# nanoporetech/vbz_compression

Measured on AMD Instinct MI355X. Metric: MB/s encode+decode, int16 signal, 1/2/4/8 MI355X vs CPU; ratio preserved, higher is better.
Workload: dtype int16

## Files before the change

### vbz_compression_amd/csrc/vbz_api.hip

```cpp
#include <hip/hip_runtime.h>

#include <cmath>
#include <cstdarg>
#include <cstdio>
#include <cstdlib>
#include <cstring>
#include <condition_variable>
#include <deque>
#include <mutex>
#include <optional>
#include <string>
#include <map>
#include <vector>

#include "../../include/vbz.h"
#include "../../include/vbz_gpu.h"
#include "vbz_kernels.h"
#include "scratch_tables.h"

using namespace vbzhip;


struct ProfEntry
{
// ... 2122 lines not shown
        return -2;
    }
    Timed t(c, "sized_layout");
    HIPCHK(c, launch_sized_layout(n, (const uint8_t*)bt->src, bt->src_off, bt->src_size, bt->src_bytes, align, raw_size, raw_off, c->stream),
           "sized layout launch");
    return 0;
}

int vbz_gpu_synth_lengths(vbz_gpu_ctx* c, uint64_t seed, uint64_t first, uint32_t n, uint32_t* out_len)
{
    if (!c) return -1;
    DeviceGuard dg(c->device);
    HIPCHK(c, launch_synth_lengths(seed, first, n, out_len, c->stream), "synth_lengths launch");
    return 0;
}

int vbz_gpu_synth_signal(vbz_gpu_ctx* c, uint64_t seed, uint64_t first, uint32_t n, void* dst, const uint64_t* off,
                         const uint32_t* len)
{
    if (!c) return -1;
    DeviceGuard dg(c->device);
    HIPCHK(c, launch_synth_signal(seed, first, n, (uint8_t*)dst, off, len, c->stream), "synth_signal launch");
    return 0;
}

int vbz_gpu_synth_u32(vbz_gpu_ctx* c, uint64_t seed, uint64_t first, uint32_t n, void* dst, const uint64_t* off, const uint32_t* len)
{
    if (!c) return -1;
    DeviceGuard dg(c->device);
    HIPCHK(c, launch_synth_u32(seed, first, n, (uint8_t*)dst, off, len, c->stream), "synth_u32 launch");
    return 0;
}

#ifdef VBZ_EXPERIMENTS
VBZ_EXPORT size_t vbz_gpu_x_plan_bytes(void) { return sizeof(EncPlan); }
VBZ_EXPORT int vbz_gpu_x_svb_handover(vbz_gpu_ctx* c, const vbz_gpu_batch* bt, void* plans_out)
{
    if (!c || !bt || !plans_out) return -1;
    DeviceGuard dg(c->device);
    const uint32_t n = bt->n_reads;
    if (n == 0) return 0;
    hipStream_t s = c->stream;
    ReadBatch rb = to_rb(bt);
    uint32_t num, den;
    svb_factor(2, true, &num, &den);
    const size_t scratch_need = (size_t)(((unsigned __int128)bt->src_bytes * num + den - 1) / den) + (size_t)n * 96 + 256;
    StageSlots m;
    if (!ensure(c, c->scratch, scratch_need) || !ensure_carved(c, c->meta, m, n) || !ensure(c, c->encplan, zstd_encode_plan_bytes(n))) return -1;
    uint64_t* const svb_off = m.svb_off;
    uint32_t *const svb_cap = m.svb_cap, *const svb_size = m.svb_size, *const gate = m.gate;
    HIPCHK(c, launch_plan_scratch(n, bt->src_size, num, den, c->scratch.cap, svb_off, svb_cap, gate, false, s), "plan launch");
    ReadBatch a = rb;
    a.dst = (uint8_t*)c->scratch.p;
    a.dst_off = svb_off;
    a.dst_cap = svb_cap;
    a.result = svb_size;
    a.gate = gate;
    HIPCHK(c, launch_svb_encode(a, 2, true, 0, false, false, nullptr, c->encplan.p, s), "svb_encode launch");
    ReadBatch cp = rb;
    cp.src = (const uint8_t*)c->scratch.p;
    cp.src_off = svb_off;
    cp.src_size = svb_size;
    cp.gate = gate;
    HIPCHK(c, launch_copy_bytes(cp, 0, s), "copy launch");
    HIPCHK(c, hipMemcpyAsync(plans_out, c->encplan.p, (size_t)n * sizeof(EncPlan), hipMemcpyDeviceToDevice, s), "plan copy");
    return 0;
}
VBZ_EXPORT int vbz_gpu_x_runs_counts(vbz_gpu_ctx* c, unsigned long long* out4, int reset)
{
    if (!c || !out4) return -1;
    DeviceGuard dg(c->device);
    HIPCHK(c, hipStreamSynchronize(c->stream), "runs counts sync");
    HIPCHK(c, zstd_fast_runs_counts(out4, reset != 0), "runs counts");
    return 0;
}
VBZ_EXPORT int vbz_gpu_x_streams_counts(vbz_gpu_ctx* c, unsigned long long* out3, int reset)
{
    if (!c || !out3) return -1;
    DeviceGuard dg(c->device);
    HIPCHK(c, hipStreamSynchronize(c->stream), "streams counts sync");
    HIPCHK(c, zstd_fast_streams_counts(out3, reset != 0), "streams counts");
    return 0;
}
#endif

void vbz_gpu_profile_enable(vbz_gpu_ctx* c, int enable)
{
    if (!c) return;
    if (!enable) drain_profile(c);
    c->profiling = enable != 0;
    if (c->half) vbz_gpu_profile_enable(c->half, enable);
}

int vbz_gpu_decode_span_paths(vbz_gpu_ctx* c, uint32_t* by_spans)
{
    if (!c) return -1;
    DeviceGuard guard(c->device);
    if (by_spans) *by_spans = 0;
    if (c->last_span_frames == 0) return 0;
    std::vector<uint32_t> redo(c->last_span_frames);
    if (hipMemcpyAsync(redo.data(), c->last_span_redo, 4ull * redo.size(), hipMemcpyDeviceToHost, c->stream) != hipSuccess) return -1;
    if (hipStreamSynchronize(c->stream) != hipSuccess) return -1;
    uint32_t nb = 0;
    for (uint32_t v : redo) nb += v == 0;
    if (by_spans) *by_spans = nb;
    return (int)c->last_span_frames;
}

static int decode_paths_one(vbz_gpu_ctx* c, uint32_t* batched, uint32_t* walked);

int vbz_gpu_decode_paths(vbz_gpu_ctx* c, uint32_t* batched, uint32_t* walked)
{
    if (!c) return -1;
    uint32_t b0 = 0, w0 = 0, b1 = 0, w1 = 0;
    const int n0 = decode_paths_one(c, &b0, &w0);
    const int n1 = (n0 >= 0 && c->last_split && c->half) ? decode_paths_one(c->half, &b1, &w1) : 0;
    if (batched) *batched = b0 + b1;
    if (walked) *walked = w0 + w1;
    return (n0 < 0 || n1 < 0) ? -1 : n0 + n1;
}

int vbz_gpu_decode_literals_ahead(vbz_gpu_ctx* c)
{
    if (!c) return -1;
    int total = 0;
    for (vbz_gpu_ctx* k : { c, (c->last_split && c->half) ? c->half : (vbz_gpu_ctx*)nullptr }) {
        if (!k || !k->last_frames || !k->last_walked || !zstd_ref_literals_enabled() || !k->reflits.p) continue;
        DeviceGuard guard(k->device);
        const uint32_t per = k->last_lit_units;
        if (per == 0) continue;
        std::vector<RefLits> lits((size_t)k->last_frames * per);
        if (hipMemcpyAsync(lits.data(), zstd_ref_lits(k->reflits.p, k->last_frames), sizeof(RefLits) * lits.size(), hipMemcpyDeviceToHost, k->stream) != hipSuccess ||
            hipStreamSynchronize(k->stream) != hipSuccess) {
            (void)hipGetLastError();
            return -1;
        }
        if (k->knobs.trace) {
            std::vector<uint32_t> sk((size_t)k->last_frames * per);
            if (hipMemcpy(sk.data(), zstd_ref_lit_skip(k->reflits.p, k->last_frames), 4 * sk.size(), hipMemcpyDeviceToHost) == hipSuccess)
                for (uint32_t u = 0; u < per; ++u) {
                    uint32_t made = 0, done = 0;
                    for (uint32_t i = 0; i < k->last_frames; ++i) {
                        made += sk[(size_t)u * k->last_frames + i] == 0;
                        done += lits[(size_t)u * k->last_frames + i].blk != 0;
                    }
                    fprintf(stderr, "vbz_hip: literals beside the walk, unit %u: %u made by the scan, %u done\n", u, made, done);
                }
        }
        for (uint32_t i = 0; i < k->last_frames; ++i) {
            bool any = false;
            for (uint32_t u = 0; u < per; ++u) any = any || lits[(size_t)u * k->last_frames + i].blk != 0;
            total += any;
        }
    }
    return total;
}

static int decode_paths_one(vbz_gpu_ctx* c, uint32_t* batched, uint32_t* walked)
{
    DeviceGuard guard(c->device);
    if (batched) *batched = 0;
    if (walked) *walked = 0;
    const uint32_t n = c->last_frames;
    if (n == 0) return 0;
    std::vector<uint32_t> redo(n);
    std::vector<RefPre> pre(c->last_walked ? n : 0);
// ... 357 lines not shown
```

### vbz_compression_amd/csrc/vbz_kernels.h

```cpp
#pragma once

#include <hip/hip_runtime.h>
#include <stdint.h>

namespace vbzhip {

constexpr uint32_t E_ZSTD = 0xFFFFFFFFu;
constexpr uint32_t E_INPUT_SIZE = 0xFFFFFFFEu;
constexpr uint32_t E_INTEGER_SIZE = 0xFFFFFFFDu;
constexpr uint32_t E_DESTINATION_SIZE = 0xFFFFFFFCu;
constexpr uint32_t E_STREAM = 0xFFFFFFFBu;
constexpr uint32_t E_VERSION = 0xFFFFFFFAu;
constexpr uint32_t E_OOM = 0xFFFFFFF9u;
constexpr uint32_t E_DEVICE = 0xFFFFFFF8u;
constexpr uint32_t E_FIRST = E_DEVICE;
constexpr uint32_t GATE_SKIP = E_FIRST - 1u;
constexpr int PHASE_SLOTS = 12;

constexpr uint32_t SIG_NONE = 0, SIG_F32 = 1, SIG_F16 = 2, SIG_BF16 = 3;
constexpr uint32_t SIG_CHUNK = 4;
constexpr uint32_t SIG_COUNT = 8;
constexpr uint32_t SIG_RANGE = 16;
constexpr uint32_t SIG_TRIM = 32;
constexpr uint32_t SIG_WINDOW = 64;
// ... 283 lines not shown
{
    hipStream_t stream = nullptr;
    hipEvent_t fork = nullptr, join = nullptr;
};
typedef SideStream FastSide;
struct SpanEncodeWork
{
    uint64_t stream_bytes = 0;
    void* meta = nullptr;
    uint8_t* tmp = nullptr;
    uint32_t shared_span_bytes = 0;
};
size_t zstd_span_meta_bytes(uint64_t stream_bytes, uint32_t n_reads, uint32_t shared_span_bytes);
uint64_t zstd_span_tmp_bytes(uint64_t stream_bytes, uint32_t n_reads);
uint32_t zstd_span_shared_bytes(uint64_t stream_bytes);
hipError_t launch_zstd_encode_spans(const ReadBatch& b, const ZstdEncodeArgs& a, const SpanEncodeWork& w, hipStream_t s);
hipError_t launch_zstd_encode_matcher(const ReadBatch& b, const ZstdEncodeArgs& a, uint32_t max_raw, const uint32_t* gate_in, uint32_t* gate_out,
                                      hipStream_t s);
hipError_t launch_zstd_decode(const ReadBatch& b, uint32_t toosmall_code, unsigned long long* dbg, const void* seq_dtables,
                              hipStream_t s);
constexpr uint32_t REF_MAXBLK = 4;
struct RefBlock
{
    uint32_t pos;
    uint32_t nseq;
    uint32_t rec_lo, rec_hi;
    uint32_t rep[3];
    uint32_t end;
};
struct RefPre
{
    uint32_t ok, nblk;
    uint32_t why;
    uint32_t tab_cycles, chain_cycles, nseq_last;
    uint32_t pad[2];
    RefBlock blk[REF_MAXBLK];
};
struct RefLits
{
    uint32_t blk, regen, csize, at;
    uint32_t tb, pcap;
    uint32_t tail, pad;
};
struct RefChains
{
    const RefPre* pre = nullptr;
    const void* recs = nullptr;
    const RefLits* lits = nullptr;
    const uint32_t* lits_pos = nullptr;
    uint32_t lits_units = 0;
};

size_t zstd_ref_pre_bytes(uint32_t n_reads);
const RefPre* zstd_ref_pre(const void* pre_meta);
size_t zstd_ref_table_bytes(uint32_t n_reads);
hipError_t launch_zstd_ref_chain(const ReadBatch& b, const uint32_t* redo, void* pre_meta, void* tables, void* recs, uint64_t recs_cap, RefChains* out,
                                 hipStream_t s);
hipError_t launch_zstd_decode_only(const ReadBatch& b, uint32_t toosmall_code, const void* seq_dtables, const uint32_t* only, RefChains chains,
                                   unsigned long long* dbg, hipStream_t s);
size_t zstd_fast_meta_bytes(uint32_t n_reads);
const RefLits* zstd_ref_lits(const void* lit_meta, uint32_t n_reads);
bool zstd_ref_literals_enabled();
const uint32_t* zstd_fast_redo(const void* meta, uint32_t n_reads);
struct RefWork
{
    void *pre = nullptr, *tables = nullptr, *recs = nullptr;
    uint64_t recs_cap = 0;
    void* lits = nullptr;
    uint32_t lit_units = 0;
};
struct FastDecodeArgs
{
    uint32_t toosmall_code = 0;
    const void* seq_dtables = nullptr;
    void* meta = nullptr;
    RefWork ref;
    unsigned long long* dbg = nullptr;
    FastSide side;
};
hipError_t launch_zstd_decode_fast(const ReadBatch& b, const FastDecodeArgs& a, hipStream_t s);
#ifdef VBZ_EXPERIMENTS
hipError_t zstd_fast_runs_counts(unsigned long long out[4], bool reset);
hipError_t zstd_fast_streams_counts(unsigned long long out[3], bool reset);
#endif
size_t zstd_ref_lit_meta_bytes(uint32_t n_reads);
uint32_t zstd_ref_lit_units();
const uint32_t* zstd_ref_lit_skip(const void* lit_meta, uint32_t n_reads);
size_t seq_dtables_bytes();
void seq_dtables_build(void* host_buffer);
struct SpanDecodeArgs
{
    uint32_t toosmall_code = 0;
    const void* seq_dtables = nullptr;
    uint64_t content_bytes = 0;
    void* meta = nullptr;
    const uint32_t* redo = nullptr;
};
size_t zstd_dspan_meta_bytes(uint64_t content_bytes, uint32_t n_reads);
hipError_t launch_zstd_decode_spans(const ReadBatch& b, SpanDecodeArgs* a, hipStream_t s);

hipError_t launch_xxh64_batch(const uint8_t* src, const uint64_t* off, const uint32_t* len, const uint32_t* gate, const uint32_t* skip, uint32_t n,
                              uint64_t* out, hipStream_t s);
hipError_t launch_xxh64_verify(const ReadBatch& b, hipStream_t s);
hipError_t launch_checksum_insert(const ReadBatch& b, const uint64_t* hash, uint32_t hdr, const uint32_t* raw_size, uint32_t integer_size, hipStream_t s);

hipError_t launch_pack_layout(uint32_t n, const uint32_t* result, const uint64_t* dst_off, const uint32_t* dst_cap, uint64_t dst_bytes, uint32_t align,
                              uint64_t* packed_off, uint32_t* packed_size, hipStream_t s);
hipError_t launch_sized_layout(uint32_t n, const uint8_t* src, const uint64_t* src_off, const uint32_t* src_size, uint64_t src_bytes, uint32_t align,
                               uint32_t* raw_size, uint64_t* raw_off, hipStream_t s);
hipError_t launch_pack_gather(uint32_t n, const uint8_t* dst, const uint64_t* dst_off, const uint64_t* packed_off, const uint32_t* packed_size,
                              uint8_t* packed, uint64_t packed_cap, hipStream_t s);

hipError_t launch_plan_scratch(uint32_t n, const uint32_t* raw_size, uint32_t mul_num, uint32_t mul_den, uint64_t limit,
                               uint64_t* off, uint32_t* cap, uint32_t* gate, bool gate_is_input, hipStream_t s);
struct ScratchPlan
{
    uint32_t num, den;
    uint64_t limit;
    uint64_t* off;
    uint32_t* cap;
    uint32_t* gate;
};
hipError_t launch_seg_plan(uint32_t n, const uint32_t* size, uint32_t unit_bytes, const uint32_t* gate, uint32_t max_segs, uint32_t* seg_first,
                           uint32_t* gate_out, const ScratchPlan* scratch, hipStream_t s);
hipError_t launch_count_nonzero(const uint32_t* a, uint32_t n, uint32_t* out, hipStream_t s);
hipError_t launch_canon_classify(uint32_t n, const uint32_t* raw_size, const uint32_t* gate, uint32_t min_bytes, uint32_t* gate_small, uint32_t* gate_large,
                                 uint32_t* counts, hipStream_t s);
struct RoutedTable
{
    uint64_t* src_off = nullptr;
    uint32_t* src_size = nullptr;
    uint64_t* dst_off = nullptr;
    uint32_t *dst_cap = nullptr, *gate = nullptr, *map = nullptr;
    float2* cal = nullptr;
    uint64_t* row = nullptr;
    uint32_t* count = nullptr;
};
struct RouteArgs
{
    const uint32_t* raw_size = nullptr;
    uint32_t min_bytes = 0, max_reads = 0;
    uint64_t max_bytes = 0;
    uint32_t* gate_small = nullptr;
    RoutedTable large;
    uint32_t* cand = nullptr;
};
hipError_t launch_route_reads(const ReadBatch& b, const RouteArgs& a, hipStream_t s);
size_t route_cand_words();
hipError_t launch_route_results(const uint32_t* l_result, const uint32_t* l_map, const uint32_t* l_count, uint32_t max_reads, uint32_t* result, hipStream_t s);
hipError_t launch_parse_sized(uint32_t n, const uint8_t* src, const uint64_t* src_off, const uint32_t* src_size,
                              const uint32_t* dst_cap, const uint32_t* gate_in, uint64_t* pay_off, uint32_t* pay_size, uint32_t* orig_size,
                              uint32_t* gate, hipStream_t s);
hipError_t launch_hand_back(const uint32_t* result, const uint8_t* src, uint32_t* host, uint32_t host_cap, uint32_t seq, uint32_t* ticket, hipStream_t s);
hipError_t launch_validate_batch(uint32_t n, const uint64_t* src_off, const uint32_t* src_size, uint64_t src_bytes, const uint64_t* dst_off,
                                 const uint32_t* dst_cap, uint64_t dst_bytes, uint32_t* gate, hipStream_t s);
hipError_t launch_signal_slots(uint32_t n, const uint64_t* dst_off, const uint32_t* dst_cap, uint32_t elem, const float* offset, const float* scale,
                               uint64_t* off16, uint32_t* cap16, float2* cal, uint32_t* gate, hipStream_t s);
hipError_t launch_chunk_slots(uint32_t n, const uint32_t* cap16, const float* offset, const float* scale, uint32_t L, uint32_t S,
                              const uint64_t* chunk_first, uint64_t chunk_rows, float2* cal, uint32_t* gate, const SignalOut* sig, hipStream_t s);
hipError_t launch_range_samples(uint32_t n, const uint32_t* samples, const uint32_t* begin, const uint32_t* end, uint32_t* range_samples, hipStream_t s);
hipError_t launch_chunk_layout(uint32_t n, const uint32_t* samples, uint32_t L, uint32_t S, uint32_t* count, uint64_t* chunk_first, hipStream_t s);
hipError_t launch_chunk_info(uint32_t n, const uint32_t* samples, uint32_t L, uint32_t S, uint32_t mode, uint32_t end_align, const uint64_t* chunk_first,
                             uint32_t* info, uint64_t info_cap, hipStream_t s);
hipError_t launch_copy_bytes(const ReadBatch& b, uint32_t hdr, hipStream_t s);
hipError_t launch_synth_lengths(uint64_t seed, uint64_t first, uint32_t n, uint32_t* out_len, hipStream_t s);
hipError_t launch_synth_signal(uint64_t seed, uint64_t first, uint32_t n, uint8_t* dst, const uint64_t* off,
// ... 59 lines not shown
```

### vbz_compression_amd/csrc/zstd_encode.hip

```cpp
#include "vbz_kernels.h"
#include "zstd_entropy.h"
#include "zstd_frame.h"

namespace vbzhip {

namespace {

constexpr int WAVE = 64;
constexpr uint32_t BLOCK_MAX = 128u << 10;
constexpr uint32_t MIN_BLOCK = 4096;
constexpr uint32_t HUF_BLOCK_MAX = 92u << 10;
constexpr uint32_t SPLIT_MIN = 2048;
constexpr int MAXBLK = 16;
#ifndef VBZ_SPAN_BLOCK_KB
#define VBZ_SPAN_BLOCK_KB 16
#endif
constexpr uint32_t SPAN_BLOCK = VBZ_SPAN_BLOCK_KB << 10;
#ifndef VBZ_SPAN_SMALL_BLOCKS
#define VBZ_SPAN_SMALL_BLOCKS 2
#endif
constexpr uint32_t SPAN_BYTES_SMALL = SPAN_BLOCK * VBZ_SPAN_SMALL_BLOCKS, SPAN_BYTES_LARGE = SPAN_BLOCK * MAXBLK;
constexpr uint32_t SPAN_LARGE_FROM = 256u << 20;
#ifndef VBZ_KEYSPAN_KB
#define VBZ_KEYSPAN_KB 8
// ... 1959 lines not shown
    }
    const uint32_t cap = b.dst_cap[r];
    uint8_t* out = b.dst + b.dst_off[r];
    if (deep_d) {
        uint32_t hint = deep_d[r];
        if (hint) {
            bool ok = false;
            if (K != 0 && src_cap && seqtab && N - K >= 8192) {
                DeepLayout dl;
                if (hint == RUN_D) hint = run_period(in + K, N - K, lane);
                ok = deep_layout(N, K, in, src_cap[r], out, cap, hdr, dl) && period_holds(in + K, N - K, hint, lane);
            }
            if (lane == 0) deep_d[r] = ok ? hint : 0u;
            if (ok) return;
        }
    }
    if ((uint64_t)hdr + 9 > cap) return;
    const uint32_t S0 = K ? K : N;
    uint32_t nrec = 0, Lit = 0;
    const uint2* rec = nullptr;
    if (src_cap && seqtab && S0 >= 256 && S0 <= BLOCK_MAX) {
        const uint32_t slot = src_cap[r];
        const uint32_t recs_all = S0 / RMIN + 2u + 2u;
        const uint64_t need = (uint64_t)N + 16 + 8ull * recs_all;
        if (need <= slot) {
            uint8_t* ws = const_cast<uint8_t*>(in) + ((slot - 8u * recs_all) & ~7u);
            PT(0);
            tokenise_runs<false>(const_cast<uint8_t*>(in), S0, reinterpret_cast<uint2*>(ws), Lit, nrec, nullptr, lane);
            __syncthreads();
            PT(1);
            rec = reinterpret_cast<const uint2*>(ws);
            if (lane == 0) {
                FP->tok_nrec = nrec;
                FP->tok_lit = Lit;
                FP->tok_done = 1;
            }
        }
    }
    if ((nrec != 0) != guess) return;
    if (nrec) {
        const uint64_t room = 24ull + 8ull * nrec;
        if (room + 4096u > cap) return;
        const uint32_t so = (uint32_t)((cap - room) & ~15ull);
        TokSeqLds& L = LL.ts;
        {
            const uint32_t* g = reinterpret_cast<const uint32_t*>(seqtab);
            uint32_t* l = reinterpret_cast<uint32_t*>(&L.seq);
            for (uint32_t i = lane; i < sizeof(SeqCTables) / 4; i += WAVE) l[i] = g[i];
        }
        wave_lds_sync();
        const uint32_t sb = encode_zero_run_sequences(L, out + so, rec, nrec, lane, 0u);
        wave_lds_sync();
        FP->cp[lane] = L.cp[lane];
        if (lane == 0) {
            FP->seqBytes = sb;
            FP->seqOff = so;
            FP->cpCount = L.cpCount;
            FP->cpSpacing = L.cpSpacing;
        }
        wave_lds_sync();
        PT(2);
    }
    const uint32_t S = nrec ? Lit : S0;
    const uint32_t nblk = nrec ? 1u : (S + T - 1) / T;
    PT(0);
    const bool ok = plan_region_table<TIMED>(LL.tb, FP, 0, in, S, nblk, nrec != 0, nrec, false, lane, tph, tlast);
    __syncthreads();
    if (ok && lane == 0) atomicOr(&pstate[r], PLAN_OPEN | PLAN_REG0 | (K == 0 ? PLAN_REG1 : 0u));
    timed_out();
}
#undef PT

#ifndef VBZ_PACK_TABLE_COPIES
#define VBZ_PACK_TABLE_COPIES 1
#endif
constexpr int PACK_COPIES = VBZ_PACK_TABLE_COPIES;
struct PackLds
{
    uint32_t ctable[PACK_COPIES * 256];
    uint32_t tree[34];
    uint32_t ssize[WAVE], sbeg[WAVE], scnt[WAVE];
    uint32_t obuf[2][OBUF_WORDS];
};

template <bool TIMED>
__device__ __forceinline__ bool pack_region(PackLds& L, const uint8_t* rin, uint32_t r0, uint8_t* out, uint32_t& opos, uint32_t limit, const uint32_t* ctable_g,
                                            const uint32_t* tree_g, uint32_t S, uint32_t nblk, uint32_t treeSize, bool seqmode, bool lastRegion,
                                            uint32_t seqBytes, uint32_t seqOff, int lane, unsigned long long (&tph)[PHASE_SLOTS], unsigned long long& tlast)
{
#define PPHASE(k) do { if (TIMED) { unsigned long long tn = __builtin_readcyclecounter(); tph[k] += tn - tlast; tlast = tn; } } while (0)
#define REDO() return false
    wave_lds_sync();
#pragma unroll
    for (int j = 0; j < 4; ++j) {
        const uint32_t e = ctable_g[lane + 64 * j];
#pragma unroll
        for (int cpy = 0; cpy < PACK_COPIES; ++cpy) L.ctable[256 * cpy + lane + 64 * j] = e;
    }
    const uint32_t* const mytable = L.ctable + 256 * (lane / (WAVE / PACK_COPIES));
    if (lane < 34) L.tree[lane] = tree_g[lane];
    const uint32_t base = S / nblk, extra = S % nblk;
    {
        const uint32_t bj = (uint32_t)(lane >> 2);
        const int q = lane & 3;
        const bool active = bj < nblk;
        uint32_t bs = 0, boff = 0;
        if (active) {
            bs = base + (bj < extra ? 1u : 0u);
            boff = bj * base + (bj < extra ? bj : extra);
        }
        const bool single = bs < 256;
        const uint32_t seg = single ? bs : (bs + 3) >> 2;
        uint32_t cnt = 0;
        if (active) {
            if (single) cnt = q == 0 ? bs : 0;
            else cnt = q < 3 ? seg : bs - 3 * seg;
        }
        L.sbeg[lane] = active ? (cnt ? boff + (uint32_t)q * seg : boff + bs) : S;
        L.scnt[lane] = cnt;
        L.ssize[lane] = 0;
    }
    for (int i = lane; i < 2 * OBUF_WORDS; i += WAVE) (&L.obuf[0][0])[i] = 0;
    wave_lds_sync();
    auto s_cnt = [&](uint32_t i) { return (uint32_t)__builtin_amdgcn_readfirstlane((int)L.scnt[i]); };
    auto s_beg = [&](uint32_t i) { return (uint32_t)__builtin_amdgcn_readfirstlane((int)L.sbeg[i]); };
    const uint32_t nb = (uint32_t)__builtin_amdgcn_readfirstlane((int)nblk);
    uint32_t st = 0;
    while (st < 4 * nb && s_cnt(st) == 0) ++st;
    uint32_t done = 0;
#if VBZ_PACK_PREFETCH
    uint32_t cur[STEP_DW], nxt[STEP_DW];
#else
    uint32_t cur[STEP_DW];
#endif
    auto load_chunk = [&](uint32_t sbeg, uint32_t scount, uint32_t dn, uint32_t (&w)[STEP_DW]) {
#pragma unroll
        for (int k = 0; k < STEP_DW; ++k) w[k] = 0;
        const int32_t room = (int32_t)(scount - dn) - STEP_LANE * lane;
        if (room > 0) {
            const uint8_t* p = rin + sbeg + room - STEP_LANE;
            const bool headroom = (uint64_t)r0 + sbeg >= (uint32_t)STEP_LANE;
            if (room >= STEP_LANE || headroom) {
                uint4 v0;
                __builtin_memcpy(&v0, p, 16);
                w[0] = v0.x; w[1] = v0.y; w[2] = v0.z; w[3] = v0.w;
            } else {
#pragma unroll
                for (int k = 0; k < STEP_LANE; ++k) {
                    const uint32_t byte = (room - STEP_LANE + k >= 0) ? (uint32_t)p[k] : 0u;
                    w[k >> 2] |= byte << (8 * (k & 3));
                }
            }
        }
    };
    auto blk_bs = [&](uint32_t j) { return base + (j < extra ? 1u : 0u); };
    auto blk_lh = [&](uint32_t j) {
        const uint32_t jbs = blk_bs(j);
        const uint32_t worst = (j == 0 ? treeSize : 0u) + 6u + ((jbs * 11u + 7u) >> 3) + 4u;
        const uint32_t big = jbs > worst ? jbs : worst;
        return 3u + (big >= 1024u ? 1u : 0u) + (big >= 16384u ? 1u : 0u);
    };
    auto block_headers = [&](uint32_t j, uint32_t at, uint32_t seqB) {
        if (lane == 0) {
            const uint32_t jbs = blk_bs(j);
            const bool jsingle = jbs < 256u;
            const uint32_t lh = blk_lh(j), tsz = j == 0 ? treeSize : 0u;
            const uint32_t s0 = L.ssize[4 * j], s1 = L.ssize[4 * j + 1], s2 = L.ssize[4 * j + 2], s3 = L.ssize[4 * j + 3];
            const uint32_t lit = tsz + (jsingle ? 0u : 6u) + s0 + s1 + s2 + s3;
            uint8_t* bp = out + at;
            const uint32_t last = (lastRegion && j + 1 == nblk) ? 1u : 0u;
            put_le(bp, ((lh + lit + seqB) << 3) | (2u << 1) | last, 3);
            const uint64_t type = (j == 0 && treeSize) ? 2 : 3;
            if (lh == 3) put_le(bp + 3, type | ((jsingle ? 0ull : 1ull) << 2) | ((uint64_t)jbs << 4) | ((uint64_t)lit << 14), 3);
            else if (lh == 4) put_le(bp + 3, type | (2ull << 2) | ((uint64_t)jbs << 4) | ((uint64_t)lit << 18), 4);
            else put_le(bp + 3, type | (3ull << 2) | ((uint64_t)jbs << 4) | ((uint64_t)lit << 22), 5);
            if (!jsingle) {
                uint8_t* tp = bp + 3 + lh + tsz;
                put_le(tp, s0, 2);
                put_le(tp + 2, s1, 2);
                put_le(tp + 4, s2, 2);
            }
        }
    };
    uint32_t ocur = opos;
    uint32_t spos = 0;
    uint32_t curblk = 0xFFFFFFFFu;
    if (st < 4 * nb) load_chunk(s_beg(st), s_cnt(st), 0, cur);
    PPHASE(1);
    uint32_t base_bits = 0;
    uint32_t flushed = 0;
    uint32_t cb = 0;
    uint32_t pend_fq = 0;
    uint8_t* pend_dst = nullptr;
    auto flush_pending = [&]() {
        uint4* pq = reinterpret_cast<uint4*>(L.obuf[cb ^ 1u]);
        for (uint32_t q = lane; q < pend_fq; q += WAVE) {
            const uint4 v = pq[q];
            pq[q] = make_uint4(0u, 0u, 0u, 0u);
            __builtin_memcpy(pend_dst + 16u * q, &v, 16);
        }
        pend_fq = 0;
    };
    while (st < 4 * nb) {
        if ((st >> 2) != curblk) {
            curblk = st >> 2;
            const uint32_t tsz = curblk == 0 ? treeSize : 0u;
            const uint32_t hl = 3u + blk_lh(curblk) + tsz + (blk_bs(curblk) < 256u ? 0u : 6u);
            if ((uint64_t)ocur + hl > limit) REDO();
            static_assert(sizeof(L.tree) <= 3 * WAVE, "a tree description is three bytes per lane at most");
#pragma unroll
            for (uint32_t i0 = 0; i0 < 3 * WAVE; i0 += WAVE) {
                const uint32_t i = i0 + (uint32_t)lane;
                if (i < tsz) out[ocur + 3u + blk_lh(curblk) + i] = reinterpret_cast<const uint8_t*>(L.tree)[i];
            }
            spos = ocur + hl;
        }
        const uint32_t scnt = s_cnt(st);
        uint8_t* sop = out + spos;
        uint32_t nst = st, ndone = done + STEP_SYMS;
        if (ndone >= scnt) {
            ndone = 0;
            ++nst;
            while (nst < 4 * nb && s_cnt(nst) == 0) ++nst;
        }
        flush_pending();
#if VBZ_PACK_PREFETCH
        if (nst < 4 * nb) load_chunk(s_beg(nst), s_cnt(nst), ndone, nxt);
#endif
        const int32_t room = (int32_t)(scnt - done) - STEP_LANE * lane;
        const int skip = room >= STEP_LANE ? 0 : (room <= 0 ? STEP_LANE : (int)(STEP_LANE - room));
        uint32_t ent[STEP_LANE];
#pragma unroll
        for (int k = 0; k < STEP_LANE; ++k) ent[k] = mytable[(cur[k >> 2] >> (8 * (k & 3))) & 0xFF];
        if (skip != 0) {
#pragma unroll
            for (int k = 0; k < STEP_LANE; ++k) ent[k] = k >= skip ? ent[k] : 0u;
        }
        uint32_t Tb = 0;
#pragma unroll
        for (int k = 0; k < STEP_LANE; ++k) Tb += ent[k];
        Tb >>= 16;
        const uint32_t incl = wave_incl_scan_u32(Tb);
        const uint32_t total = (uint32_t)__builtin_amdgcn_readlane((int)incl, 63);
        const uint32_t allbits = base_bits + total;
        const uint32_t fq = allbits >> 7;
        if ((uint64_t)spos + flushed + 16ull * fq + 24 > limit) REDO();
        PPHASE(2);
        {
            const uint32_t pos = base_bits + incl - Tb;
            uint32_t word = pos >> 5;
            uint32_t accbits = pos & 31;
            uint64_t acc = 0;
#pragma unroll
            for (int k = STEP_LANE - 1; k >= 0; k -= 2) {
                const uint32_t e1 = ent[k], e0 = ent[k - 1];
                const uint32_t l1 = e1 >> 16, l0 = e0 >> 16;
                const uint64_t pair = (uint64_t)((e1 & 0xFFFFu) | ((e0 & 0xFFFFu) << l1));
                acc |= pair << accbits;
                accbits += l1 + l0;
                if (accbits >= 32) {
                    atomicOr(&L.obuf[cb][word], (uint32_t)acc);
                    acc >>= 32;
                    accbits -= 32;
                    ++word;
                }
            }
            if (acc) atomicOr(&L.obuf[cb][word], (uint32_t)acc);
        }
        wave_lds_sync();
        PPHASE(3);
        {
            uint4* obq = reinterpret_cast<uint4*>(L.obuf[cb]);
            uint4* nbq = reinterpret_cast<uint4*>(L.obuf[cb ^ 1u]);
            if (lane == 0) {
                const uint4 c = obq[fq];
                obq[fq] = make_uint4(0u, 0u, 0u, 0u);
                nbq[0] = c;
            }
            pend_fq = fq;
            pend_dst = sop + flushed;
            cb ^= 1u;
        }
        flushed += 16u * fq;
        base_bits = allbits & 127u;
        wave_lds_sync();
        PPHASE(4);
        if (nst != st) {
            const uint32_t nbytes = (base_bits + 1 + 7) >> 3;
            {
                uint4* obq = reinterpret_cast<uint4*>(L.obuf[cb]);
                const uint4 c = obq[0];
                const uint32_t cw[4] = { c.x, c.y, c.z, c.w };
                uint32_t mine = cw[(lane >> 2) & 3];
                if ((uint32_t)(lane >> 2) == (base_bits >> 5)) mine |= 1u << (base_bits & 31u);
                if ((uint32_t)lane < nbytes) sop[flushed + lane] = (uint8_t)(mine >> (8 * (lane & 3)));
                wave_lds_sync();
                if (lane == 0) {
                    obq[0] = make_uint4(0u, 0u, 0u, 0u);
                    L.ssize[st] = flushed + nbytes;
                }
            }
            spos += flushed + nbytes;
            base_bits = 0;
            flushed = 0;
            if ((nst >> 2) != curblk && !seqmode) {
                wave_lds_sync();
                if ((uint64_t)spos + 1 > limit) REDO();
                if (lane == 0) out[spos] = 0;
                block_headers(curblk, ocur, 1u);
                ocur = spos + 1u;
            }
        }
#if VBZ_PACK_PREFETCH
#pragma unroll
        for (int k = 0; k < STEP_DW; ++k) cur[k] = nxt[k];
#else
        if (nst < 4 * nb) load_chunk(s_beg(nst), s_cnt(nst), ndone, cur);
#endif
        st = nst;
        done = ndone;
        PPHASE(5);
    }
    flush_pending();
    if (seqmode && curblk != 0xFFFFFFFFu) {
        wave_lds_sync();
        if ((uint64_t)spos + seqBytes > seqOff) REDO();
        for (uint32_t i = 16u * (uint32_t)lane; i < seqBytes; i += 16u * WAVE) {
            uint4 v;
            __builtin_memcpy(&v, out + seqOff + i, 16);
            if (i + 16u <= seqBytes) __builtin_memcpy(out + spos + i, &v, 16);
            else {
                const uint32_t w[4] = { v.x, v.y, v.z, v.w };
                for (uint32_t k = i; k < seqBytes; ++k) out[spos + k] = (uint8_t)(w[(k - i) >> 2] >> (8 * ((k - i) & 3)));
            }
        }
        wave_lds_sync();
        block_headers(curblk, ocur, seqBytes);
        ocur = spos + seqBytes;
    }
    opos = ocur;
    return true;
#undef PPHASE
#undef REDO
}

template <bool TIMED>
__global__ __launch_bounds__(WAVE, TIMED ? VBZ_ENC_PACK_WAVES_TIMED : VBZ_ENC_PACK_WAVES) void zstd_pack_kernel(ReadBatch b, const uint32_t* orig_size, uint32_t key_elem, const uint32_t* key_bytes,
                                                                             uint32_t hdr, uint32_t trailers, const EncPlan* plans, uint32_t* redo,
                                                                             unsigned long long* dbg_)
{
    unsigned long long* const dbg = TIMED ? dbg_ : nullptr;
    __shared__ __attribute__((aligned(16))) PackLds L;
    unsigned long long tph[PHASE_SLOTS] = {};
    unsigned long long tlast = TIMED ? __builtin_readcyclecounter() : 0;
#define PPHASE(k) do { if (TIMED) { unsigned long long tn = __builtin_readcyclecounter(); tph[k] += tn - tlast; tlast = tn; } } while (0)
    const int lane = threadIdx.x;
    const uint32_t r = blockIdx.x;
    if (redo[r] != PLAN_READY) return;
#define REDO()                          \
    do {                                \
        if (lane == 0) redo[r] = 0;     \
        return;                         \
    } while (0)
    const uint32_t N = b.src_size[r];
    const uint32_t cap = b.dst_cap[r];
    const uint8_t* in = b.src + b.src_off[r];
    uint8_t* out = b.dst + b.dst_off[r];
    const EncPlan* FP = &plans[r];
    uint32_t K = 0;
    if (N >= SPLIT_MIN) {
        if (key_bytes) K = key_bytes[r];
        else if (key_elem) K = (orig_size[r] / key_elem + 3u) >> 2;
        if (K >= N) K = 0;
    }
    const uint32_t seqBytes = FP->seqBytes, seqOff = FP->seqOff;
    const uint32_t limit = seqBytes ? seqOff : cap;
    uint32_t opos = 0;
    if ((uint64_t)hdr + 9 > limit) REDO();
    if (lane == 0) {
        if (hdr) put_le(out, orig_size[r], 4);
        uint8_t* p = out + hdr;
        put_le(p, ZSTD_MAGIC, 4);
        if (N < 256) { p[4] = 0x20; p[5] = (uint8_t)N; }
        else if (N < 65536 + 256) { p[4] = 0x60; put_le(p + 5, N - 256, 2); }
        else { p[4] = 0xA0; put_le(p + 5, N, 4); }
    }
    opos = hdr + 5 + (N < 256 ? 1 : (N < 65536 + 256 ? 2 : 4));
    PPHASE(0);
    for (int region = 0; region < 2; ++region) {
        if (region == 1 && K == 0) break;
        const uint32_t r0 = region == 0 ? 0u : K;
        const uint32_t r1 = region == 0 ? (K ? K : N) : N;
        const EncRegionPlan* P = &FP->reg[region];
        const uint32_t S = P->S, Sh = P->Sh;
        const uint32_t opos_region = opos;
        int rlane = lane;
        asm volatile("" : "+v"(rlane));
        if (!pack_region<TIMED>(L, in + r0, r0, out, opos, limit, P->ctable, P->tree, S, P->nblk, P->treeSize, P->seqmode != 0, r1 == N, seqBytes, seqOff, rlane,
                                tph, tlast))
            REDO();
        if (Sh != S && opos - opos_region > S + (S >> 6) + 256u) REDO();
        PPHASE(6);
    }
    if (FP->cpCount != 0 && (trailers & 1u)) {
        const uint32_t count = FP->cpCount, tb = 8u + 4u + 4u * count + 4u;
// ... 360 lines not shown
            }
        };
        for (uint32_t c = tid; c < nchunk; c += 4 * 256) {
            uint32_t w[4] = { 0u, 0u, 0u, 0u };
#pragma unroll
            for (int q = 0; q < 4; ++q)
                if (c + 256u * q < nchunk) __builtin_memcpy(&w[q], data + 16u * (c + 256u * q), 4);
#pragma unroll
            for (int q = 0; q < 4; ++q)
                if (c + 256u * q < nchunk) look_up(16u * (c + 256u * q), w[q]);
        }
    }
    __syncthreads();
    if (tid < WAVE) {
        const uint32_t hint = best == 0xFFFFFFFFu ? ((!placed && SD >= PP_P0 + PP_TRIES * PP_SHIFT + 48u) ? RUN_D : 0u) : best;
        uint32_t D = 0;
        if (hint) {
            const uint8_t* in = b.src + b.src_off[r];
            DeepLayout dl;
            const uint32_t h2 = hint == RUN_D ? run_period(in + K, SD, tid) : hint;
            if (deep_layout(N, K, in, src_cap[r], b.dst + b.dst_off[r], b.dst_cap[r], hdr, dl) && period_holds(in + K, SD, h2, tid)) D = h2;
        }
        if (tid == 0) {
            deep_d[r] = D;
            gate_out[r] = D ? GATE_SKIP : (gate ? gate[r] : 0u);
        }
    }
}

}

hipError_t launch_zstd_encode(const ReadBatch& b, const ZstdEncodeArgs& a, hipStream_t s)
{
    const uint32_t* const orig_size = a.key.orig_size;
    const uint32_t key_elem = a.key.key_elem, hdr = a.hdr;
    const uint32_t* const key_bytes = a.key.key_bytes;
    const uint32_t* const src_cap = a.runs.src_cap;
    const bool trailers = a.trailers;
    uint32_t* const deep_d = a.deep_d;
    void* const plan_meta = a.plan_meta;
    bool staged = a.staged, pre_filled = a.pre_filled;
    if (!plan_meta) staged = pre_filled = false;
    const uint32_t tr = (trailers ? ENC_TRAILERS : 0u) | (pre_filled ? ENC_PRE_FILLED : 0u);
    if (b.n_reads == 0) return hipSuccess;
    const SeqCTables* st = reinterpret_cast<const SeqCTables*>(a.runs.seq_tables);
#ifdef VBZ_EXPERIMENTS
    unsigned long long *const dbg = a.dbg.frame, *const plan_dbg = a.dbg.plan, *const pack_dbg = a.dbg.pack;
    if (dbg && !plan_meta) {
        hipLaunchKernelGGL((zstd_encode_kernel<true, false>), dim3(b.n_reads), dim3(WAVE), 0, s, b, orig_size, key_elem, key_bytes, hdr, dbg,
                           src_cap, st, nullptr, nullptr, nullptr, nullptr, nullptr, tr, nullptr, nullptr, nullptr, SpanShared{});
        return hipGetLastError();
    }
#endif
    EncPlan* plans = reinterpret_cast<EncPlan*>(plan_meta);
    uint32_t* redo = plans ? reinterpret_cast<uint32_t*>(plans + b.n_reads) : nullptr;
    if (staged && src_cap && st) {
        (void)hipMemsetAsync(redo, 0, 4ull * b.n_reads, s);
#ifdef VBZ_EXPERIMENTS
        if (plan_dbg)
            hipLaunchKernelGGL(zstd_plan_kernel<true>, dim3(2 * b.n_reads), dim3(WAVE), 0, s, b, orig_size, key_elem, key_bytes, hdr, src_cap, st, deep_d, plans,
                               redo, pre_filled ? 1u : 0u, plan_dbg);
        else
#endif
        hipLaunchKernelGGL(zstd_plan_kernel<false>, dim3(2 * b.n_reads), dim3(WAVE), 0, s, b, orig_size, key_elem, key_bytes, hdr, src_cap, st, deep_d, plans,
                           redo, pre_filled ? 1u : 0u, (unsigned long long*)nullptr);
#ifdef VBZ_EXPERIMENTS
        if (pack_dbg)
            hipLaunchKernelGGL(zstd_pack_kernel<true>, dim3(b.n_reads), dim3(WAVE), 0, s, b, orig_size, key_elem, key_bytes, hdr, tr, plans, redo, pack_dbg);
        else
#endif
        hipLaunchKernelGGL(zstd_pack_kernel<false>, dim3(b.n_reads), dim3(WAVE), 0, s, b, orig_size, key_elem, key_bytes, hdr, tr, plans, redo, (unsigned long long*)nullptr);
    } else {
        redo = nullptr;
    }
    hipLaunchKernelGGL((zstd_encode_kernel<false, false>), dim3(b.n_reads), dim3(WAVE), 0, s, b, orig_size, key_elem, key_bytes, hdr, nullptr,
                       src_cap, st, nullptr, nullptr, nullptr, nullptr, nullptr, tr, deep_d, redo ? plans : nullptr, redo, SpanShared{});
    if (deep_d)
        hipLaunchKernelGGL((zstd_encode_kernel<false, true>), dim3(b.n_reads), dim3(WAVE), 0, s, b, orig_size, key_elem, key_bytes, hdr, nullptr,
                           src_cap, st, nullptr, nullptr, nullptr, nullptr, nullptr, tr, deep_d, redo ? plans : nullptr, nullptr, SpanShared{});
    return hipGetLastError();
}

size_t zstd_encode_plan_bytes(uint32_t n_reads) { return (size_t)n_reads * (sizeof(EncPlan) + 4) + 256; }

hipError_t launch_zstd_encode_matcher(const ReadBatch& b, const ZstdEncodeArgs& a, uint32_t max_raw, const uint32_t* gate_in, uint32_t* gate_out,
                                      hipStream_t s)
{
    if (b.n_reads == 0) return hipSuccess;
    const uint32_t* const orig_size = a.key.orig_size;
    const uint32_t key_elem = a.key.key_elem, hdr = a.hdr;
    const uint32_t* const src_cap = a.runs.src_cap;
    const bool trailers = a.trailers;
    uint32_t* const deep_d = a.deep_d;
    const SeqCTables* st = reinterpret_cast<const SeqCTables*>(a.runs.seq_tables);
    hipLaunchKernelGGL(period_probe_kernel, dim3(b.n_reads), dim3(256), 0, s, b, orig_size, key_elem, hdr, src_cap, max_raw, gate_in, deep_d, gate_out);
    ReadBatch g = b;
    g.gate = gate_in;
    hipLaunchKernelGGL((zstd_encode_kernel<false, true>), dim3(b.n_reads), dim3(WAVE), 0, s, g, orig_size, key_elem, (const uint32_t*)nullptr, hdr,
                       (unsigned long long*)nullptr, src_cap, st, nullptr, nullptr, nullptr, nullptr, nullptr, trailers ? 1u : 0u, deep_d, nullptr, nullptr, SpanShared{});
    return hipGetLastError();
}

uint32_t zstd_span_shared_bytes(uint64_t stream_bytes) { return stream_bytes < SHSPAN_BATCH_FROM ? SHSPAN_BYTES : 0u; }

static uint32_t span_max_spans(uint64_t stream_bytes, uint32_t n_reads)
{
    const uint64_t v = stream_bytes / (KEYSPAN_BYTES_SHARED / 2) + 4ull * n_reads + 1;
    return v > 0x7FFFFFF0ull ? 0u : (uint32_t)v;
}

uint64_t zstd_span_tmp_bytes(uint64_t stream_bytes, uint32_t n_reads)
{
    return stream_bytes + (stream_bytes >> 7) + stream_bytes * 8u / RMIN + (uint64_t)span_max_spans(stream_bytes, n_reads) * 2048u + 4096u;
}

struct SpanTables
{
    SpanRegion* regions;
    EncSpan* spans;
    uint32_t *first, *count, *size, *trail, *dst;
    SpanTables(void* meta, uint32_t n_reads, uint32_t max_spans, bool shared)
    {
        MetaCarver sm(meta);
        regions = shared ? reinterpret_cast<SpanRegion*>(sm.take<uint8_t>((size_t)n_reads * sizeof(SpanRegion))) : nullptr;
        spans = reinterpret_cast<EncSpan*>(sm.take<uint8_t>((size_t)max_spans * sizeof(EncSpan)));
        first = sm.take<uint32_t>((size_t)n_reads + 1);
        count = sm.take<uint32_t>(1);
        size = sm.take<uint32_t>(max_spans);
        trail = sm.take<uint32_t>(max_spans);
        dst = sm.take<uint32_t>(max_spans);
    }
};

size_t zstd_span_meta_bytes(uint64_t stream_bytes, uint32_t n_reads, uint32_t shared_span_bytes)
{
    const uint32_t max_spans = span_max_spans(stream_bytes, n_reads);
    if (!max_spans) return 0;
    return (size_t)max_spans * (sizeof(EncSpan) + 12) + ((size_t)n_reads + 2) * 4 + 256 + (shared_span_bytes ? (size_t)n_reads * sizeof(SpanRegion) + 64 : 0);
}

hipError_t launch_zstd_encode_spans(const ReadBatch& b, const ZstdEncodeArgs& a, const SpanEncodeWork& w, hipStream_t s)
{
    if (b.n_reads == 0) return hipSuccess;
    const uint32_t max_spans = span_max_spans(w.stream_bytes, b.n_reads);
    if (!max_spans || !w.meta) return hipErrorInvalidValue;
    const SpanTables T(w.meta, b.n_reads, max_spans, w.shared_span_bytes != 0);
    const uint32_t* const orig_size = a.key.orig_size;
    const uint32_t key_elem = a.key.key_elem, hdr = a.hdr, shared_span_bytes = w.shared_span_bytes;
    const uint32_t* const src_cap = a.runs.src_cap;
    const void* const seq_tables = a.runs.seq_tables;
    const bool index_trailer = a.trailers;
    uint8_t* const span_tmp = w.tmp;
    const uint64_t span_tmp_bytes = zstd_span_tmp_bytes(w.stream_bytes, b.n_reads);
    EncSpan* const spans = T.spans;
    SpanRegion* const regions = T.regions;
    uint32_t *const span_first = T.first, *const span_count = T.count, *const span_size = T.size, *const span_trail = T.trail, *const span_dst = T.dst;
    hipLaunchKernelGGL(zstd_span_plan_kernel, dim3(1), dim3(1024), 0, s, b.n_reads, b.src_size, orig_size, key_elem, b.gate,
                       (src_cap && seq_tables) ? 1u : 0u, max_spans, span_tmp_bytes, spans, span_first, span_count, regions, shared_span_bytes);
    const SpanShared shared = { regions, max_spans, regions ? shared_span_bytes : 0u };
    if (regions) hipLaunchKernelGGL(zstd_span_count_kernel, dim3((max_spans + 3) / 4), dim3(256), 0, s, b, spans, span_count, regions);
    if (regions)
        hipLaunchKernelGGL((zstd_encode_kernel<false, false, true>), dim3(max_spans + b.n_reads), dim3(WAVE), 0, s, b, orig_size, key_elem, nullptr, hdr, nullptr, src_cap,
                           reinterpret_cast<const SeqCTables*>(seq_tables), spans, span_count, span_tmp, span_size, span_trail, index_trailer ? 1u : 0u,
                           nullptr, nullptr, nullptr, shared);
    else
        hipLaunchKernelGGL((zstd_encode_kernel<false, false>), dim3(max_spans), dim3(WAVE), 0, s, b, orig_size, key_elem, nullptr, hdr, nullptr, src_cap,
// ... 15 lines not shown
```

Baseline: 663,600.

## Pack the tail of one Huffman stream together with the next stream's head in one wave step

The Huffman pack loop used to spend a full 64-lane step on each stream's final partial chunk, leaving lanes idle. It now lets the idle lanes start on the next stream, or the next block, within the same step. It places the end-of-stream bit, leaves a byte-aligned hole for any block header, and then moves the next stream's write position. The goal is fewer wave steps per read in the encode pack kernel. The cost is more complex lookahead planning, extra readlane work and a new layout invariant, which is checked by a static_assert on the LDS buffer; experiment-only step counters are also added.

```diff
diff --git a/vbz_compression_amd/csrc/vbz_api.hip b/vbz_compression_amd/csrc/vbz_api.hip
--- a/vbz_compression_amd/csrc/vbz_api.hip
+++ b/vbz_compression_amd/csrc/vbz_api.hip
@@ -2228,6 +2228,14 @@
     HIPCHK(c, zstd_fast_streams_counts(out3, reset != 0), "streams counts");
     return 0;
 }
+VBZ_EXPORT int vbz_gpu_x_pack_counts(vbz_gpu_ctx* c, unsigned long long* out4, int reset)
+{
+    if (!c || !out4) return -1;
+    DeviceGuard dg(c->device);
+    HIPCHK(c, hipStreamSynchronize(c->stream), "pack counts sync");
+    HIPCHK(c, zstd_pack_counts(out4, reset != 0), "pack counts");
+    return 0;
+}
 #endif
 
 void vbz_gpu_profile_enable(vbz_gpu_ctx* c, int enable)
diff --git a/vbz_compression_amd/csrc/vbz_kernels.h b/vbz_compression_amd/csrc/vbz_kernels.h
--- a/vbz_compression_amd/csrc/vbz_kernels.h
+++ b/vbz_compression_amd/csrc/vbz_kernels.h
@@ -389,6 +389,7 @@
 #ifdef VBZ_EXPERIMENTS
 hipError_t zstd_fast_runs_counts(unsigned long long out[4], bool reset);
 hipError_t zstd_fast_streams_counts(unsigned long long out[3], bool reset);
+hipError_t zstd_pack_counts(unsigned long long out[4], bool reset);
 #endif
 size_t zstd_ref_lit_meta_bytes(uint32_t n_reads);
 uint32_t zstd_ref_lit_units();
diff --git a/vbz_compression_amd/csrc/zstd_encode.hip b/vbz_compression_amd/csrc/zstd_encode.hip
--- a/vbz_compression_amd/csrc/zstd_encode.hip
+++ b/vbz_compression_amd/csrc/zstd_encode.hip
@@ -2065,6 +2065,12 @@
     uint32_t ssize[WAVE], sbeg[WAVE], scnt[WAVE];
     uint32_t obuf[2][OBUF_WORDS];
 };
+constexpr int PACK_HOLE_MAX = 1 + 3 + 5 + 6;
+static_assert(((127 + STEP_SYMS * 11 + 1 + 7 + 8 * PACK_HOLE_MAX) >> 7) + 1 <= OBUF_WORDS / 4 && OBUF_WORDS % 4 == 0, "a packing step's bits overrun the LDS bit buffer");
+
+#ifdef VBZ_EXPERIMENTS
+__device__ unsigned long long pack_counts[4];
+#endif
 
 template <bool TIMED>
 __device__ __forceinline__ bool pack_region(PackLds& L, const uint8_t* rin, uint32_t r0, uint8_t* out, uint32_t& opos, uint32_t limit, const uint32_t* ctable_g,
@@ -2108,18 +2114,47 @@
     auto s_cnt = [&](uint32_t i) { return (uint32_t)__builtin_amdgcn_readfirstlane((int)L.scnt[i]); };
     auto s_beg = [&](uint32_t i) { return (uint32_t)__builtin_amdgcn_readfirstlane((int)L.sbeg[i]); };
     const uint32_t nb = (uint32_t)__builtin_amdgcn_readfirstlane((int)nblk);
+    const uint32_t nstr = 4 * nb;
     uint32_t st = 0;
-    while (st < 4 * nb && s_cnt(st) == 0) ++st;
+    while (st < nstr && s_cnt(st) == 0) ++st;
     uint32_t done = 0;
 #if VBZ_PACK_PREFETCH
     uint32_t cur[STEP_DW], nxt[STEP_DW];
 #else
     uint32_t cur[STEP_DW];
 #endif
-    auto load_chunk = [&](uint32_t sbeg, uint32_t scount, uint32_t dn, uint32_t (&w)[STEP_DW]) {
+    auto plan_step = [&](uint32_t s, uint32_t dn, uint32_t& la_, uint32_t& ns_, uint32_t& nd_) {
+        la_ = WAVE;
+        ns_ = s;
+        nd_ = 0;
+        if (s >= nstr) return;
+        const uint32_t rem = s_cnt(s) - dn;
+        if (rem > (uint32_t)STEP_SYMS) {
+            nd_ = dn + STEP_SYMS;
+            return;
+        }
+        ++ns_;
+        while (ns_ < nstr && s_cnt(ns_) == 0) ++ns_;
+        const uint32_t lanes = (rem + STEP_LANE - 1) / STEP_LANE, slots = STEP_LANE * (WAVE - lanes);
+        if (ns_ >= nstr || slots == 0) return;
+        const uint32_t bcnt = s_cnt(ns_);
+        if ((ns_ >> 2) == (s >> 2) ? bcnt > slots : (!seqmode && bcnt >= (uint32_t)STEP_SYMS)) {
+            la_ = lanes;
+            nd_ = slots;
+        }
+    };
+    auto load_step = [&](uint32_t s, uint32_t dn, uint32_t la_, uint32_t ns_, uint32_t (&w)[STEP_DW]) {
 #pragma unroll
         for (int k = 0; k < STEP_DW; ++k) w[k] = 0;
-        const int32_t room = (int32_t)(scount - dn) - STEP_LANE * lane;
+        uint32_t sbeg = s_beg(s);
+        int32_t room = (int32_t)(s_cnt(s) - dn) - STEP_LANE * lane;
+        if (la_ < (uint32_t)WAVE) {
+            const uint32_t bbeg = s_beg(ns_), bcnt = s_cnt(ns_);
+            if ((uint32_t)lane >= la_) {
+                sbeg = bbeg;
+                room = (int32_t)bcnt - STEP_LANE * (lane - (int)la_);
+            }
+        }
         if (room > 0) {
             const uint8_t* p = rin + sbeg + room - STEP_LANE;
             const bool headroom = (uint64_t)r0 + sbeg >= (uint32_t)STEP_LANE;
@@ -2168,13 +2203,18 @@
     uint32_t ocur = opos;
     uint32_t spos = 0;
     uint32_t curblk = 0xFFFFFFFFu;
-    if (st < 4 * nb) load_chunk(s_beg(st), s_cnt(st), 0, cur);
+    uint32_t la, nst, ndone;
+    plan_step(st, 0, la, nst, ndone);
+    if (st < nstr) load_step(st, 0, la, nst, cur);
     PPHASE(1);
     uint32_t base_bits = 0;
-    uint32_t flushed = 0;
+    uint32_t wp = 0;
     uint32_t cb = 0;
     uint32_t pend_fq = 0;
     uint8_t* pend_dst = nullptr;
+#ifdef VBZ_EXPERIMENTS
+    uint32_t steps = 0;
+#endif
     auto flush_pending = [&]() {
         uint4* pq = reinterpret_cast<uint4*>(L.obuf[cb ^ 1u]);
         for (uint32_t q = lane; q < pend_fq; q += WAVE) {
@@ -2184,7 +2224,7 @@
         }
         pend_fq = 0;
     };
-    while (st < 4 * nb) {
+    while (st < nstr) {
         if ((st >> 2) != curblk) {
             curblk = st >> 2;
             const uint32_t tsz = curblk == 0 ? treeSize : 0u;
@@ -2197,20 +2237,18 @@
                 if (i < tsz) out[ocur + 3u + blk_lh(curblk) + i] = reinterpret_cast<const uint8_t*>(L.tree)[i];
             }
             spos = ocur + hl;
-        }
-        const uint32_t scnt = s_cnt(st);
-        uint8_t* sop = out + spos;
-        uint32_t nst = st, ndone = done + STEP_SYMS;
-        if (ndone >= scnt) {
-            ndone = 0;
-            ++nst;
-            while (nst < 4 * nb && s_cnt(nst) == 0) ++nst;
-        }
+            wp = spos;
+        }
+        const uint32_t rem = s_cnt(st) - done;
+        const bool joined = la < (uint32_t)WAVE;
+        uint32_t la2, nst2, ndone2;
+        plan_step(nst, ndone, la2, nst2, ndone2);
         flush_pending();
 #if VBZ_PACK_PREFETCH
-        if (nst < 4 * nb) load_chunk(s_beg(nst), s_cnt(nst), ndone, nxt);
+        if (nst < nstr) load_step(nst, ndone, la2, nst2, nxt);
 #endif
-        const int32_t room = (int32_t)(scnt - done) - STEP_LANE * lane;
+        const bool inB = (uint32_t)lane >= la;
+        const int32_t room = inB ? STEP_LANE : (int32_t)rem - STEP_LANE * lane;
         const int skip = room >= STEP_LANE ? 0 : (room <= 0 ? STEP_LANE : (int)(STEP_LANE - room));
         uint32_t ent[STEP_LANE];
 #pragma unroll
@@ -2225,12 +2263,22 @@
         Tb >>= 16;
         const uint32_t incl = wave_incl_scan_u32(Tb);
         const uint32_t total = (uint32_t)__builtin_amdgcn_readlane((int)incl, 63);
-        const uint32_t allbits = base_bits + total;
+        uint32_t off = base_bits;
+        uint32_t allbits = base_bits + total;
+        uint32_t enda = 0, bstart = 0;
+        if (joined) {
+            const uint32_t incla = (uint32_t)__builtin_amdgcn_readlane((int)incl, (int)la - 1);
+            enda = base_bits + incla;
+            const uint32_t hole = (nst >> 2) != curblk ? 1u + 3u + blk_lh(nst >> 2) + 6u : 0u;
+            bstart = ((enda + 8u) & ~7u) + 8u * hole;
+            if (inB) off = bstart - incla;
+            allbits = bstart + total - incla;
+        }
         const uint32_t fq = allbits >> 7;
-        if ((uint64_t)spos + flushed + 16ull * fq + 24 > limit) REDO();
+        if ((uint64_t)wp + 16ull * fq + 24 > limit) REDO();
         PPHASE(2);
         {
-            const uint32_t pos = base_bits + incl - Tb;
+            const uint32_t pos = off + incl - Tb;
             uint32_t word = pos >> 5;
             uint32_t accbits = pos & 31;
             uint64_t acc = 0;
@@ -2249,9 +2297,11 @@
                 }
             }
             if (acc) atomicOr(&L.obuf[cb][word], (uint32_t)acc);
+            if (joined && lane == 0) atomicOr(&L.obuf[cb][enda >> 5], 1u << (enda & 31u));
         }
         wave_lds_sync();
         PPHASE(3);
+        const uint32_t wp0 = wp;
         {
             uint4* obq = reinterpret_cast<uint4*>(L.obuf[cb]);
             uint4* nbq = reinterpret_cast<uint4*>(L.obuf[cb ^ 1u]);
@@ -2261,14 +2311,23 @@
                 nbq[0] = c;
             }
             pend_fq = fq;
-            pend_dst = sop + flushed;
+            pend_dst = out + wp0;
             cb ^= 1u;
         }
-        flushed += 16u * fq;
+        wp += 16u * fq;
         base_bits = allbits & 127u;
         wave_lds_sync();
         PPHASE(4);
-        if (nst != st) {
+        if (joined) {
+            const uint32_t aend = wp0 + ((enda + 8u) >> 3);
+            if (lane == 0) L.ssize[st] = aend - spos;
+            spos = wp0 + (bstart >> 3);
+            if ((nst >> 2) != curblk) {
+                block_headers(curblk, ocur, 1u);
+                ocur = aend + 1u;
+                curblk = nst >> 2;
+            }
+        } else if (nst != st) {
             const uint32_t nbytes = (base_bits + 1 + 7) >> 3;
             {
                 uint4* obq = reinterpret_cast<uint4*>(L.obuf[cb]);
@@ -2276,16 +2335,16 @@
                 const uint32_t cw[4] = { c.x, c.y, c.z, c.w };
                 uint32_t mine = cw[(lane >> 2) & 3];
                 if ((uint32_t)(lane >> 2) == (base_bits >> 5)) mine |= 1u << (base_bits & 31u);
-                if ((uint32_t)lane < nbytes) sop[flushed + lane] = (uint8_t)(mine >> (8 * (lane & 3)));
+                if ((uint32_t)lane < nbytes) out[wp + lane] = (uint8_t)(mine >> (8 * (lane & 3)));
                 wave_lds_sync();
                 if (lane == 0) {
                     obq[0] = make_uint4(0u, 0u, 0u, 0u);
-                    L.ssize[st] = flushed + nbytes;
+                    L.ssize[st] = wp + nbytes - spos;
                 }
             }
-            spos += flushed + nbytes;
+            spos = wp + nbytes;
+            wp = spos;
             base_bits = 0;
-            flushed = 0;
             if ((nst >> 2) != curblk && !seqmode) {
                 wave_lds_sync();
                 if ((uint64_t)spos + 1 > limit) REDO();
@@ -2298,12 +2357,30 @@
 #pragma unroll
         for (int k = 0; k < STEP_DW; ++k) cur[k] = nxt[k];
 #else
-        if (nst < 4 * nb) load_chunk(s_beg(nst), s_cnt(nst), ndone, cur);
+        if (nst < nstr) load_step(nst, ndone, la2, nst2, cur);
 #endif
         st = nst;
         done = ndone;
+        la = la2;
+        nst = nst2;
+        ndone = ndone2;
+#ifdef VBZ_EXPERIMENTS
+        ++steps;
+#endif
         PPHASE(5);
     }
+#ifdef VBZ_EXPERIMENTS
+    {
+        uint32_t mine = (L.scnt[lane] + STEP_SYMS - 1) / STEP_SYMS;
+        for (int d = 32; d > 0; d >>= 1) mine += __shfl_xor(mine, d);
+        if (lane == 0) {
+            atomicAdd(&pack_counts[0], (unsigned long long)steps);
+            atomicAdd(&pack_counts[1], (unsigned long long)steps * STEP_SYMS);
+            atomicAdd(&pack_counts[2], (unsigned long long)S);
+            atomicAdd(&pack_counts[3], (unsigned long long)mine);
+        }
+    }
+#endif
     flush_pending();
     if (seqmode && curblk != 0xFFFFFFFFu) {
         wave_lds_sync();
@@ -2830,6 +2907,18 @@
 }
 
 size_t zstd_encode_plan_bytes(uint32_t n_reads) { return (size_t)n_reads * (sizeof(EncPlan) + 4) + 256; }
+
+#ifdef VBZ_EXPERIMENTS
+hipError_t zstd_pack_counts(unsigned long long out[4], bool reset)
+{
+    hipError_t e = hipMemcpyFromSymbol(out, HIP_SYMBOL(pack_counts), sizeof(pack_counts));
+    if (e == hipSuccess && reset) {
+        const unsigned long long zero[4] = { 0, 0, 0, 0 };
+        e = hipMemcpyToSymbol(HIP_SYMBOL(pack_counts), zero, sizeof(zero));
+    }
+    return e;
+}
+#endif
 
 hipError_t launch_zstd_encode_matcher(const ReadBatch& b, const ZstdEncodeArgs& a, uint32_t max_raw, const uint32_t* gate_in, uint32_t* gate_out,
                                       hipStream_t s)
```

Result: no change. 670,100, median of 6 (+1.0%).
